# Darkkey/erlamsa

Measured on AMD Instinct MI355X. Metric: mutated_MB_per_s, higher is better.
Workload: dtype u8 (byte edits) + f64 (AS183 draws)

## Files before the change

### erlamsa_amd/csrc/eh_fuse_red.h

```cpp
#pragma once

namespace eh {

constexpr uint32_t FR_NONE = 0xFFFFFFFFu;
constexpr uint32_t FR_MAX_PERIOD = 1u << 16;
constexpr int FR_LEVELS = 4;

EH_DEV uint64_t fr_ld8(cbptr S, uint32_t q, uint32_t len) {
  uint64_t by = 0;
  if (q + 8 <= len) by = ldg8(S + q);
  else { for (uint32_t k = 0; k < 8; k++) if (q + k < len) by |= (uint64_t)S[q + k] << (8 * k); }
  return by;
}
EH_DEV uint32_t fr_peek_rounds(const Rng& r) {
  const uint32_t l = (uint32_t)EH_LANE;
  double x = rng_peek(r, l + 1u) * 8.0;
  unsigned long long z = __ballot((uint32_t)x == 0u);
  return z ? (uint32_t)__builtin_ctzll(z) : 64u;
}
__device__ __noinline__ uint32_t fr_run_fwd(cbptr S, uint32_t i0, uint32_t p, uint32_t n) {
  const uint32_t l = (uint32_t)EH_LANE;
  const uint32_t lim = n - p;
  for (uint32_t base = i0;; base += 1024) {
    const uint32_t q = base + 16u * l;
    uint32_t mp = FR_NONE;
    if (q + 16 <= lim) {
      uint4 a, b;
      a = ldg16(S + q); b = ldg16(S + q + p);
      const uint32_t x[4] = {a.x ^ b.x, a.y ^ b.y, a.z ^ b.z, a.w ^ b.w};
#pragma unroll
      for (int k = 3; k >= 0; k--) if (x[k]) mp = q + 4u * (uint32_t)k + ((uint32_t)__builtin_ctz(x[k]) >> 3);
    } else {
      for (uint32_t k = 0; k < 16; k++) { if (q + k >= lim || S[q + k] != S[q + k + p]) { mp = q + k; break; } }
    }
    unsigned long long hit = __ballot(mp != FR_NONE);
    if (hit) return (uint32_t)__builtin_amdgcn_readlane((int)mp, (int)__builtin_ctzll(hit));
  }
}
__device__ __noinline__ uint32_t fr_run_bwd(cbptr S, uint32_t i0, uint32_t p) {
  const uint32_t l = (uint32_t)EH_LANE;
  for (uint32_t hi = i0;; hi -= 1024) {
    uint32_t mp = FR_NONE;
    const uint32_t top = 16u * l < hi ? hi - 16u * l : 0u, bot = 16u * (l + 1u) < hi ? hi - 16u * (l + 1u) : 0u;
    if (top - bot == 16u) {
      uint4 a, b;
      a = ldg16(S + bot); b = ldg16(S + bot + p);
      const uint32_t x[4] = {a.x ^ b.x, a.y ^ b.y, a.z ^ b.z, a.w ^ b.w};
#pragma unroll
      for (int k = 0; k < 4; k++) if (x[k]) mp = bot + 4u * (uint32_t)k + ((31u - (uint32_t)__builtin_clz(x[k])) >> 3);
    } else {
      for (uint32_t k = bot; k < top; k++) if (S[k] != S[k + p]) mp = k;
    }
    unsigned long long hit = __ballot(mp != FR_NONE);
    if (hit) return (uint32_t)__builtin_amdgcn_readlane((int)mp, (int)__builtin_ctzll(hit)) + 1u;
    if (hi <= 1024) return 0;
  }
}
__device__ __noinline__ uint32_t fr_find8(cbptr S, uint32_t from, uint32_t lim, uint32_t n, uint64_t key) {
  const uint32_t l = (uint32_t)EH_LANE;
  if (n < 8) return FR_NONE;
  if (lim > n - 7) lim = n - 7;
  for (uint32_t base = from; base < lim; base += 1024) {
    const uint32_t q = base + 16u * l;
    uint64_t w0 = 0, w1 = 0, w2 = 0;
    if (q + 24 <= n) { w0 = ldg8(S + q); w1 = ldg8(S + q + 8); w2 = ldg8(S + q + 16); }
    else if (q < lim) { w0 = fr_ld8(S, q, n); w1 = fr_ld8(S, q + 8, n); w2 = fr_ld8(S, q + 16, n); }
    uint32_t first = 16;
#pragma unroll
    for (int k = 15; k >= 0; k--) {
      const uint64_t lo = k < 8 ? w0 : w1, hi = k < 8 ? w1 : w2;
      const int sh = 8 * (k & 7);
      const uint64_t win = sh ? (lo >> sh) | (hi << (64 - sh)) : lo;
      if (win == key && q + (uint32_t)k < lim) first = (uint32_t)k;
    }
    unsigned long long hit = __ballot(first < 16);
    if (hit) { int src = (int)__builtin_ctzll(hit); return base + 16u * (uint32_t)src + (uint32_t)__builtin_amdgcn_readlane((int)first, src); }
  }
  return FR_NONE;
}
__device__ __noinline__ bool fr_find_cut(cbptr S, uint32_t n, uint32_t R, uint32_t* cu, uint32_t* cD, uint32_t* cP = nullptr) {
  uint32_t bestD = 0, bestU = 0, blo = 0, bhi = 0, bestP = 0;
  if (n < 4096) return false;
  bool any = false;
  for (uint32_t ai = 0; ai < 7; ai++) {
    const uint32_t a = ai == 0 ? 4u : ai == 1 ? 2u : ai == 2 ? 6u : ai == 3 ? 1u : ai == 4 ? 3u : ai == 5 ? 5u : 7u;
    if (ai == 3 && !any) break;
    const uint32_t x = (uint32_t)(((uint64_t)n * a) >> 3);
    if (x + 8 > n) continue;
    if (bestD && x >= blo && x < bhi) continue;
    const uint64_t key = fr_ld8(S, x, n);
    uint32_t y = x + 1;
    for (int tries = 0; tries < 4; tries++) {
      const uint32_t far = x + 1u + FR_MAX_PERIOD < n ? x + 1u + FR_MAX_PERIOD : n;
      y = fr_find8(S, y, far, n, key);
      if (y == FR_NONE) break;
      any = true;
      const uint32_t p = y - x;
      const uint32_t hi = fr_run_fwd(S, x, p, n), lo = fr_run_bwd(S, x, p);
      const uint32_t u = lo + p, b = hi + p;
      if (b > u + R && b - u - R >= p) {
        const uint32_t D = (b - R - u) / p * p;
        if (D > bestD) { bestD = D; bestU = u; blo = lo; bhi = b; bestP = p; }
      }
      if (bestD >= n / 2) break;
      y++;
    }
    if (bestD >= n / 2) break;
  }
  if (bestD < 2048 || bestD < n / 8) return false;
  *cu = bestU; *cD = bestD;
  if (cP) *cP = bestP;
  return true;
}
__device__ __noinline__ cbptr fr_reduce(Ctx&, cbptr S, uint32_t* n, uint32_t R) {
  EH_CTX;
  uint32_t u = 0, D = 0, len = *n;
  if (!fr_find_cut(S, len, R, &u, &D)) return S;
  bptr C = ws_alloc(c, (uint64_t)len - D + 16);
  if (!C) return nullptr;
  wave_copy(C, S, u);
  wave_copy(C + u, S + u + D, len - u - D);
  len -= D;
  wave_sync();
  for (int lv = 1; lv < FR_LEVELS; lv++) {
    if (!fr_find_cut(C, len, R, &u, &D)) break;
    wave_sync();
    wave_move_down(C + u, C + u + D, len - u - D);
    len -= D;
    wave_sync();
// ... 60 lines not shown
```

### erlamsa_amd/csrc/eh_sgml.h

```cpp
#pragma once
#include "eh_doc.h"

namespace eh {

enum { E_LT = 1, E_GT, E_WS, E_EQ, E_SL, E_SQ, E_DQ, E_DASH, E_QM, E_BANG, E_SLGT, E_QGT, E_CMTEND, E_SPACE };
constexpr uint32_t ES_WS = (1u << E_WS) | (1u << E_SPACE);
constexpr uint32_t ES_EV = ES_WS | (1u << E_GT) | (1u << E_EQ);
constexpr uint32_t ES_STOP = ES_EV | (1u << E_SLGT);
constexpr uint32_t ES_DASH = (1u << E_DASH) | (1u << E_CMTEND);
EH_DEV uint32_t sg_class(uint32_t b) {
  const uint64_t t0 = ((uint64_t)E_WS << 36) | ((uint64_t)E_WS << 40) | ((uint64_t)E_WS << 52);
  const uint64_t t2 = ((uint64_t)E_SPACE << 0) | ((uint64_t)E_BANG << 4) | ((uint64_t)E_DQ << 8) | ((uint64_t)E_SQ << 28) | ((uint64_t)E_DASH << 52) | ((uint64_t)E_SL << 60);
  const uint64_t t3 = ((uint64_t)E_LT << 48) | ((uint64_t)E_EQ << 52) | ((uint64_t)E_GT << 56) | ((uint64_t)E_QM << 60);
  uint64_t t = b < 16 ? t0 : (b < 32 ? 0ull : (b < 48 ? t2 : t3));
  return b < 64 ? (uint32_t)((t >> (4 * (b & 15))) & 15) : 0u;
}

__constant__ uint8_t c_sglit[24] = {'<', '>', ' ', '=', '\'', '"', '<', '/', ' ', '/', '>', '<', '?', '?', '>', '<', '!', '<', '!', '-', '-', '-', '-', '>'};
enum { SL_LT = 0, SL_GT = 1, SL_SP = 2, SL_EQ = 3, SL_SQ = 4, SL_DQ = 5, SL_LTSL = 6, SL_SPSLGT = 8, SL_LTQ = 11, SL_QGT = 13, SL_LTBANG = 15, SL_CMT = 17, SL_CMTEND = 21 };
EH_DEV cbptr sglit(int k) { return (cbptr)&c_sglit[k]; }

enum { TK_OPEN = 1, TK_CLOSE = 2, TK_SC = 3, TK_TEXT = 4, TK_BANG = 5, TK_COMMENT = 6, TK_QUE = 7, TK_KIND = 0xFF, TF_EMPTY = 0x100, TF_PAIRED = 0x200 };
struct SgTok { uint32_t kind, p0, np, na, nb, par0, npar; int32_t match; };
struct SgParam { uint32_t na, nb, va, vb, delim, pad; };
// ... 224 lines not shown
        R.va = pos + 1; R.vb = EV(jq) >> 4; R.delim = cv == E_SQ ? 1u : 2u;
        pos = R.vb + 1; ei = jq + 1;
      } else {
        const uint32_t ju = find_stop(ei);
        if (ju >= nev || bail) break;
        R.va = pos; R.vb = EV(ju) >> 4; pos = R.vb; ei = ju;
      }
      skipws();
    }
    if (bail) break;
    R.term = 0; R.npos = pos; R.nei = ei; R.nws = ws_sp ? 1u : 0u;
  } while (false);
  R.reach = reach;
  return R;
}

__device__ __noinline__ int sgml_tokenize(Ctx&, cbptr H, uint32_t L, SgDoc* out) {
  EH_CTX;
  const int l = EH_LANE;
#ifdef EH_PROF
  const uint64_t ph1_t0 = __builtin_readcyclecounter();
#endif
  wptr ev = (wptr)ws_alloc(c, ((uint64_t)L + 80) * 4);
  if (!ev) return -3;
  uint32_t nev = 0, nlt = 0, nstop = 0;
  for (uint32_t tb = 0; tb < L; tb += 1024) {
    uint32_t i0 = tb + 16u * (uint32_t)l;
    uint8_t b[18];
    if (i0 + 18 <= L) { uint4 v = ldg16(H + i0); __builtin_memcpy(b, &v, 16); b[16] = H[i0 + 16]; b[17] = H[i0 + 17]; }
    else { for (uint32_t k = 0; k < 18; k++) b[k] = i0 + k < L ? H[i0 + k] : 0; }
    uint32_t cls[16]; uint32_t cnt = 0, lts = 0, stops = 0;
#pragma unroll
    for (uint32_t k = 0; k < 16; k++) {
      uint32_t x = b[k];
      uint32_t cl = i0 + k < L ? sg_class(x) : 0u;
      if (cl == E_SL && b[k + 1] == '>') cl = E_SLGT;
      if (cl == E_QM && b[k + 1] == '>') cl = E_QGT;
      if (cl == E_DASH && b[k + 1] == '-' && b[k + 2] == '>') cl = E_CMTEND;
      cls[k] = cl; cnt += cl ? 1u : 0u; lts += cl == E_LT ? 1u : 0u; stops += (cl == E_WS || cl == E_SPACE || cl == E_GT || cl == E_EQ || cl == E_SL || cl == E_SLGT) ? 1u : 0u;
    }
    uint32_t inc = wave_incl_scan(cnt);
    uint32_t o = nev + inc - cnt;
#pragma unroll
    for (uint32_t k = 0; k < 16; k++) if (cls[k]) ev[o++] = ((i0 + k) << 4) | cls[k];
    nev += (uint32_t)__builtin_amdgcn_readlane((int)inc, 63);
    nlt += lts; nstop += stops;
  }
  nlt = wave_sum(nlt); nstop = wave_sum(nstop);
#ifdef EH_PROF
  uint64_t sub_t0 = __builtin_readcyclecounter();
#define SG_SUB0() do { sub_t0 = __builtin_readcyclecounter(); } while (0)
#define SG_SUB(k) do { uint64_t n_ = __builtin_readcyclecounter(); if (l == 0) { atomicAdd(&c.p->prof[2 * (k)], (unsigned long long)(n_ - sub_t0)); atomicAdd(&c.p->prof[2 * (k) + 1], 1ull); } sub_t0 = n_; } while (0)
#define SG_CNT(k, v) do { if (l == 0) { atomicAdd(&c.p->prof[2 * (k)], (unsigned long long)(v)); atomicAdd(&c.p->prof[2 * (k) + 1], 1ull); } } while (0)
  if (l == 0) { atomicAdd(&c.p->prof[2 * 117], (unsigned long long)(sub_t0 - ph1_t0)); atomicAdd(&c.p->prof[2 * 117 + 1], 1ull); atomicAdd(&c.p->prof[2 * 119], (unsigned long long)nev); atomicAdd(&c.p->prof[2 * 119 + 1], (unsigned long long)L); }
  uint64_t tz_t0 = __builtin_readcyclecounter();
#define SG_TZ(k) do { uint64_t n_ = __builtin_readcyclecounter(); if (l == 0) { atomicAdd(&c.p->prof[2 * (k)], (unsigned long long)(n_ - tz_t0)); atomicAdd(&c.p->prof[2 * (k) + 1], 1ull); } tz_t0 = n_; } while (0)
#else
#define SG_TZ(k) do {} while (0)
#define SG_SUB0() do {} while (0)
#define SG_SUB(k) do {} while (0)
#define SG_CNT(k, v) do {} while (0)
#endif
  if (nlt == 0) return -1;
  uint32_t cap_tok = 2 * nlt + 8, cap_par = nstop + 8;
  uint64_t cap_pc = 4ull * cap_tok + (uint64_t)SG_PARPCS * cap_par + nlt + 32;
  EH_G SgTok* tok = (EH_G SgTok*)ws_alloc(c, (uint64_t)cap_tok * sizeof(SgTok));
  EH_G SgParam* par = (EH_G SgParam*)ws_alloc(c, (uint64_t)cap_par * sizeof(SgParam));
  EH_G Piece* pc = (EH_G Piece*)ws_alloc(c, cap_pc * sizeof(Piece));
  if (!tok || !par || !pc) return -3;
  wave_sync();
  uint32_t ntok = 0, npar = 0, npc = 0;

  constexpr uint32_t SG_EVC = 4096, SG_EVBACK = 512;
  uint32_t cbase = 0xFFFFFFFFu;
  uint32_t bev = 0, bbase = 0xFFFFFFFFu;
  uint32_t reach_ev = 0;
  auto need = [&](uint32_t i) {
    if (bbase != 0xFFFFFFFFu && i >= bbase && i < bbase + 64) return;
    bbase = i & ~63u;
    if (bbase + 64 > reach_ev) reach_ev = bbase + 64;
    if (cbase == 0xFFFFFFFFu || bbase < cbase || bbase + 64 > cbase + SG_EVC) {
      cbase = bbase > SG_EVBACK ? bbase - SG_EVBACK : 0u;
      lanes_sync();
      for (uint32_t k0 = 0; k0 < SG_EVC; k0 += 256) {
        uint32_t v[4];
#pragma unroll
        for (int u = 0; u < 4; u++) { uint32_t j = cbase + k0 + 64u * (uint32_t)u + (uint32_t)l; v[u] = j < nev ? ev[j] : 0u; }
#pragma unroll
        for (int u = 0; u < 4; u++) g_fuse_lds[k0 + 64u * (uint32_t)u + (uint32_t)l] = v[u];
      }
      lanes_sync();
    }
    bev = g_fuse_lds[bbase - cbase + (uint32_t)l];
  };
  auto find = [&](uint32_t from, uint32_t set) -> uint32_t {
    while (from < nev) {
      need(from);
      unsigned long long m = __ballot(((set >> (bev & 15u)) & 1u) != 0 && bbase + (uint32_t)l >= from && bbase + (uint32_t)l < nev);
      if (m) return bbase + (uint32_t)__builtin_ctzll(m);
      from = bbase + 64;
    }
    return nev;
  };
  auto evget = [&](uint32_t i) -> uint32_t { need(i); return (uint32_t)__builtin_amdgcn_readlane((int)bev, (int)(i - bbase)); };
  uint32_t ff_gt = nev, ff_qgt = nev, ff_cmt = nev, ff_sq = nev, ff_dq = nev;
  auto find1 = [&](uint32_t from, uint32_t cls, uint32_t& ff) -> uint32_t {
    if (from >= ff) return nev;
// ... 1014 lines not shown
```

### erlamsa_amd/csrc/eh_text.h

```cpp
#pragma once
#include "eh_device.h"

namespace eh {

template <class Pred>
EH_DEV uint32_t tile_mask(cbptr p, uint32_t n, uint32_t tile_base, Pred pred) {
  uint32_t i0 = tile_base + 16u * (uint32_t)EH_LANE;
  if (i0 >= n) return 0;
  uint32_t cnt = n - i0 < 16 ? n - i0 : 16;
  uint8_t b[16];
  if (cnt == 16) { uint4 v = ldg16(p + i0); __builtin_memcpy(b, &v, 16); }
  else { for (uint32_t k = 0; k < 16; k++) b[k] = k < cnt ? p[i0 + k] : 0; }
  uint32_t prev = i0 > 0 ? p[i0 - 1] : 256u;
  uint32_t m = 0;
#pragma unroll
  for (uint32_t k = 0; k < 16; k++) {
    if (k < cnt && pred((uint32_t)b[k], prev)) m |= 1u << k;
    prev = b[k];
  }
  return m;
}
EH_DEV uint32_t wave_incl_scan(uint32_t v) {
  const int l = EH_LANE;
#pragma unroll
  for (int d = 1; d < 64; d <<= 1) { uint32_t t = __shfl_up(v, d); if (l >= d) v += t; }
  return v;
}
EH_DEV uint32_t wave_sum(uint32_t v) {
#pragma unroll
  for (int d = 32; d > 0; d >>= 1) v += __shfl_xor(v, d);
  return uni(v);
}
template <class Pred>
EH_DEV uint32_t wave_count(cbptr p, uint32_t n, Pred pred) {
  uint32_t c = 0;
  for (uint32_t tb = 0; tb < n; tb += 1024) c += __popc(tile_mask(p, n, tb, pred));
  return wave_sum(c);
}
template <class Pred>
EH_DEV uint32_t wave_find_kth(cbptr p, uint32_t n, uint32_t k, Pred pred) {
  uint32_t before = 0;
  for (uint32_t tb = 0; tb < n; tb += 1024) {
    uint32_t m = tile_mask(p, n, tb, pred);
    uint32_t inc = wave_incl_scan(__popc(m));
    uint32_t tile_total = uni((uint32_t)__shfl(inc, 63));
    if (k < before + tile_total) {
      uint32_t kk = k - before;
      bool mine = inc > kk && inc - __popc(m) <= kk;
      unsigned long long who = __ballot(mine);
      int src = (int)__builtin_ctzll(who);
      uint32_t pos = 0;
      if (mine) {
        uint32_t r = kk - (inc - __popc(m));
        uint32_t mm = m;
        for (uint32_t t = 0; t < r; t++) mm &= mm - 1;
        pos = tb + 16u * (uint32_t)EH_LANE + (uint32_t)__builtin_ctz(mm);
      }
      return uni((uint32_t)__shfl(pos, src));
    }
    before += tile_total;
  }
  return n;
}
template <class Pred>
EH_DEV void wave_collect(cbptr p, uint32_t n, uint32_t r0, uint32_t r1, wptr out, Pred pred) {
  uint32_t before = 0;
  for (uint32_t tb = 0; tb < n && before < r1; tb += 1024) {
    uint32_t m = tile_mask(p, n, tb, pred);
    uint32_t inc = wave_incl_scan(__popc(m));
    uint32_t rank = before + inc - __popc(m);
    uint32_t mm = m;
    while (mm) {
      uint32_t bit = (uint32_t)__builtin_ctz(mm); mm &= mm - 1;
      if (rank >= r0 && rank < r1) out[rank - r0] = tb + 16u * (uint32_t)EH_LANE + bit;
      rank++;
    }
    before += uni((uint32_t)__shfl(inc, 63));
  }
  wave_sync();
}

EH_DEV bool binarish(cbptr p, uint32_t n) {
  const int l = EH_LANE;
  uint32_t mine = (uint32_t)l < n && l < 11 ? p[l] : 0;
  uint32_t b[11];
#pragma unroll
  for (int k = 0; k < 11; k++) b[k] = (uint32_t)__builtin_amdgcn_readlane((int)mine, k);
#pragma unroll
  for (uint32_t pos = 0; pos <= 8; pos++) {
    uint32_t rem = n > pos ? n - pos : 0;
    if (rem >= 3 && b[pos] == 0xEF && b[pos + 1] == 0xBB && b[pos + 2] == 0xBF) return false;
    if (rem >= 2 && b[pos] == 0xFE && b[pos + 1] == 0x0F) return false;
    if (pos == 8) return false;
    if (rem == 0) return false;
    if (b[pos] == 0) return true;
    if (b[pos] & 128) return true;
  }
  return false;
}

struct Pieces {
  uint64_t p[6]; uint32_t n[6]; uint32_t rep[6]; int k;
};
EH_DEV void pc_init(Pieces& q) { q.k = 0; }
EH_DEV void pc_add(Pieces& q, cbptr p, uint32_t n, uint32_t rep = 1) { q.p[q.k] = (uint64_t)p; q.n[q.k] = n; q.rep[q.k] = rep; q.k++; }
EH_DEV bool pc_emit(Ctx& c, const Pieces& q) {
  uint64_t total = 0;
#pragma unroll
  for (int i = 0; i < 6; i++) if (i < q.k) total += (uint64_t)q.n[i] * q.rep[i];
  if (total > 0xFFFFFFF0ull) { EH_SET_OVERFLOW(c, 701); return false; }
  bptr dst = ws_alloc(c, total);
  if (!dst) return false;
  uint64_t pos = 0;
#pragma unroll
  for (int i = 0; i < 6; i++) if (i < q.k) {
    if (q.rep[i] == 1) wave_copy(dst + pos, (cbptr)q.p[i], q.n[i]);
    else wave_fill_periodic(dst + pos, (cbptr)q.p[i], q.n[i], (uint64_t)q.n[i] * q.rep[i]);
    pos += (uint64_t)q.n[i] * q.rep[i];
  }
  wave_sync();
  c.r_kind = R_NEW; c.r_ptr = dst; c.r_len = (uint32_t)total;
  return true;
}

struct IsNl { EH_DEV bool operator()(uint32_t b, uint32_t) const { return b == 10; } };

struct LineIdx {
  cbptr p; uint32_t L, nnl, N;
};
EH_DEV void li_init(LineIdx& li, cbptr p, uint32_t L) {
// ... 497 lines not shown
```

### erlamsa_amd/csrc/eh_tree.h

```cpp
#pragma once
#include "eh_lex.h"

namespace eh {

struct TNode { uint32_t open, close, pend, pad; };

EH_DEV uint32_t usual_delim_close(uint32_t c) {
  switch (c) { case 40: return 41; case 91: return 93; case 60: return 62; case 123: return 125; case 34: return 34; case 39: return 39; }
  return 0;
}
struct DelimCls {
  EH_DEV uint32_t operator()(uint32_t b) const {
    switch (b) { case 40: return 1; case 41: return 2; case 91: return 3; case 93: return 4; case 60: return 5; case 62: return 6;
                 case 123: return 7; case 125: return 8; case 34: return 9; case 39: return 10; }
    return 0;
  }
};
EH_DEV uint32_t delim_close_code(uint32_t code) { return code == 9 ? 9u : (code == 10 ? 10u : code + 1); }
EH_DEV bool delim_is_opener(uint32_t code) { return code == 1 || code == 3 || code == 5 || code == 7 || code == 9 || code == 10; }
EH_DEV bool delim_bit(uint32_t b, uint32_t w1, uint32_t w23) { uint32_t m = b < 32 ? 0u : (b < 64 ? w1 : (b < 128 ? w23 : 0u)); return (m >> (b & 31u)) & 1u; }
struct IsOpener { EH_DEV bool operator()(uint32_t b, uint32_t) const { return delim_bit(b, (1u << 2) | (1u << 7) | (1u << 8) | (1u << 28), 1u << 27); } };

#ifndef EH_TREE_S
#define EH_TREE_S 32
#endif
constexpr uint32_t TL_S = EH_TREE_S;
constexpr uint32_t TL_SP = TL_S + 4;
constexpr uint32_t TL_COD = 0;
constexpr uint32_t TL_LNK = TL_COD + 16 * TL_SP;
constexpr uint32_t TL_STK = TL_LNK + 16 * TL_SP;
constexpr uint32_t TL_TOP = TL_STK + 32 * TL_S;
constexpr uint32_t TL_ESC = TL_TOP + 64 * TL_S;
constexpr uint32_t TL_TAIL = 4 * TL_S;
constexpr uint32_t TL_SEQ_MIN = 1024, TL_SEQ_MAX = 65536;
static_assert(TL_S >= 8 && TL_S <= 32 && TL_S % 4 == 0, "tree_parse: per-run event masks are 32 bits wide");
static_assert(TL_ESC + 16 * TL_SP <= EH_FUSE_LDS_WORDS, "g_fuse_lds too small for the lane batches of tree_parse");
EH_DEV uint8_t* tl_bytes() { return reinterpret_cast<uint8_t*>(g_fuse_lds); }
EH_DEV uint16_t* tl_stack() { return reinterpret_cast<uint16_t*>(g_fuse_lds + TL_STK); }
#ifdef EH_PROF
#define TR_PH(k) do { uint64_t now_ = __builtin_readcyclecounter(); if (EH_LANE == 0) { atomicAdd(&c.p->prof[2 * (70 + (k))], (unsigned long long)(now_ - tph)); atomicAdd(&c.p->prof[2 * (70 + (k)) + 1], 1ull); } tph = now_; } while (0)
#define TR_ST(k, v) do { if (EH_LANE == 0) { atomicAdd(&c.p->prof[2 * (70 + (k))], (unsigned long long)(v)); atomicAdd(&c.p->prof[2 * (70 + (k)) + 1], 1ull); } } while (0)
#else
#define TR_PH(k) do { } while (0)
#define TR_ST(k, v) do { } while (0)
#endif
#ifdef HIPEMU
extern "C" { inline unsigned long long eh_emu_tree_lanes[5] = {0, 0, 0, 0, 0}; }
#define TL_COUNT(i, v) do { if (EH_LANE == 0) eh_emu_tree_lanes[i] += (v); } while (0)
#else
#define TL_COUNT(i, v) do { } while (0)
#endif
struct IsDelim { EH_DEV bool operator()(uint32_t b, uint32_t) const { return delim_bit(b, (1u << 2) | (1u << 7) | (1u << 8) | (1u << 9) | (1u << 28) | (1u << 30), (1u << 27) | (1u << 29)); } };
EH_DEV void delim_tile_masks(cbptr p, uint32_t n, uint32_t tile_base, uint32_t& md, uint32_t& mo, uint32_t& mq) {
  md = 0; mo = 0; mq = 0;
  uint32_t i0 = tile_base + 16u * (uint32_t)EH_LANE;
  if (i0 >= n) return;
  uint32_t cnt = n - i0 < 16 ? n - i0 : 16;
  uint8_t b[16];
  if (cnt == 16) { uint4 v = ldg16(p + i0); __builtin_memcpy(b, &v, 16); }
  else { for (uint32_t k = 0; k < 16; k++) b[k] = k < cnt ? p[i0 + k] : 0; }
#pragma unroll
  for (uint32_t k = 0; k < 16; k++) {
    if (IsDelim()((uint32_t)b[k], 0)) md |= 1u << k;
    if (IsOpener()((uint32_t)b[k], 0)) mo |= 1u << k;
#ifdef EH_PROF
    if (b[k] == 34 || b[k] == 39) mq |= 1u << k;
#endif
  }
}
__device__ __noinline__ int tree_parse(Ctx&, cbptr H, uint32_t L, EH_G TNode** out) {
  EH_CTX;
  const int l = EH_LANE;
#ifdef EH_PROF
  uint64_t tph = __builtin_readcyclecounter();
#endif
  uint32_t nev = 0, nopen = 0, nquote = 0;
  for (uint32_t tb = 0; tb < L; tb += 1024) { uint32_t md, mo, mq; delim_tile_masks(H, L, tb, md, mo, mq); nev += __popc(md); nopen += __popc(mo); nquote += __popc(mq); }
  nev = wave_sum(nev); nopen = wave_sum(nopen);
#ifdef EH_PROF
  nquote = wave_sum(nquote);
#endif
  EH_G TNode* tab = (EH_G TNode*)ws_alloc(c, (uint64_t)(nopen + 1) * sizeof(TNode));
  wptr spill = (wptr)ws_alloc(c, (uint64_t)(nopen + 64) * 4);
  wptr evp = (wptr)ws_alloc(c, (uint64_t)(nev + 64) * 4);
  if (!tab || !spill || !evp) return -1;
  if (nopen >= (1u << 24)) { EH_SET_OVERFLOW(c, 801); return -1; }
  TR_PH(10);
  wave_collect(H, L, 0, nev, evp, IsDelim());
  TR_PH(11); TR_ST(15, nev);
  for (uint32_t i = (uint32_t)l; i < nopen + 1; i += 64) tab[i].close = 0xFFFFFFFFu;
  wave_sync();
  uint32_t stk = 0;
  uint32_t sp = 0, sbase = 0;
  uint32_t top = 0;
  uint32_t orank = 0;
  auto rs_refill = [&]() {
    uint32_t up = (uint32_t)__shfl_up((int)stk, 32);
    sbase -= 32;
    stk = l < 32 ? spill[sbase + l] : up;
  };
  auto rs_spill = [&]() {
    if (l < 32) spill[sbase + l] = stk;
    stk = (uint32_t)__shfl_down((int)stk, 32);
    sbase += 32;
  };
  auto rs_pop = [&]() {
    sp--;
    if (sp > 0) {
      if (sp == sbase) rs_refill();
      top = (uint32_t)__builtin_amdgcn_readlane((int)stk, (int)(sp - 1 - sbase));
    }
  };
  auto rs_push = [&](uint32_t ent) {
    if (sp - sbase == 64) rs_spill();
    if ((uint32_t)l == sp - sbase) stk = ent;
    top = ent; sp++;
  };
  const bool lanes_on = !(c.p->flags & EH_FLAG_TREE_NO_LANES) && nev >= 8 * TL_S;
  uint32_t seq_left = 0, seq_len = TL_SEQ_MIN;
  uint32_t nlane = 0;
  if (lanes_on) { TL_COUNT(3, 1); TL_COUNT(4, nev); }
  uint32_t eb = 0;
  while (eb < nev) {
    eb = uni(eb); sp = uni(sp); sbase = uni(sbase); top = uni(top); orank = uni(orank); seq_left = uni(seq_left); seq_len = uni(seq_len);
    if (!lanes_on || seq_left > 0 || nev - eb < TL_TAIL) {
      uint32_t mycode = eb + (uint32_t)l < nev ? DelimCls()((uint32_t)H[evp[eb + l]]) : 0;
      mycode |= delim_is_opener(mycode) ? (0x100u | (delim_close_code(mycode) << 16)) : 0u;
      uint32_t cnt = nev - eb < 64 ? nev - eb : 64;
      const unsigned long long opm = __ballot((mycode & 0x100u) != 0);
      uint32_t npush = 0, nclose = 0;
// ... 150 lines not shown
        const uint32_t rb = ob + (uint32_t)__popc(okm & ((1u << sj) - 1));
        for (uint32_t e2 = 0; e2 < rem; e2++) {
          const uint32_t code = (uint32_t)__builtin_amdgcn_readlane((int)mc, (int)e2);
          if (sp > 0 && (code & 255u) == (top & 255u)) {
            if ((uint32_t)l == nclose) { cs = top >> 8; ce = ev0 + sj + e2; }
            nclose++;
            rs_pop();
            if (nclose == 64) w_flush();
          } else if (code & 0x100u) {
            const uint32_t parent = sp > 0 ? top >> 8 : 0xFFFFFFFFu;
            const uint32_t slot = rb + (uint32_t)__popcll(opm & ((1ull << e2) - 1));
            if ((uint32_t)l == npush) { ps = slot; pe = ev0 + sj + e2; pp = parent; }
            npush++;
            rs_push((slot << 8) | (code >> 16));
            if (npush == 64) w_flush();
          }
        }
        nseq += rem;
      }
      if (l == k) topout = sp > 0 ? top >> 8 : 0xFFFFFFFFu;
    }
    w_flush();
    lanes_sync();
    {
      const unsigned long long below = items & ((1ull << l) - 1);
      const uint32_t t = (uint32_t)__shfl((int)topout, below ? 63 - (int)__builtin_clzll(below) : 0);
      if (!((items >> l) & 1ull)) topin = below ? t : top0;
    }
    {
      const uint32_t lb = 4 * TL_LNK + (uint32_t)l * TL_SP, ev0 = eb + (uint32_t)l * TL_S;
      uint32_t m = cm;
      while (m) {
        const uint32_t j = (uint32_t)__builtin_ctz(m); m &= m - 1;
        const uint32_t jo = tl_bytes()[lb + j], lp = tl_bytes()[lb + jo];
        const uint32_t slot = obase + (uint32_t)__popc(om & ((1u << jo) - 1));
        uint32_t par;
        if (lp != 255u) par = obase + (uint32_t)__popc(om & ((1u << lp) - 1));
        else { const uint32_t e = (uint32_t)__popc(em & ((1u << jo) - 1)); par = e ? g_fuse_lds[TL_TOP + (uint32_t)l * TL_S + e - 1] : topin; }
        tab[slot].open = ev0 + jo; tab[slot].close = ev0 + j; tab[slot].pend = par;
      }
    }
    orank += (uint32_t)__builtin_amdgcn_readlane((int)oinc, 63);
    eb += committed;
    nlane += committed - nseq; TL_COUNT(0, committed - nseq); TL_COUNT(1, 1);
    if (2 * nseq > committed) { TL_COUNT(2, 1); seq_left = seq_len; if (seq_len < TL_SEQ_MAX) seq_len *= 2; }
    else if (seq_len > TL_SEQ_MIN) seq_len /= 2;
  }
  wave_sync();
  TR_PH(12);
#ifdef EH_PROF
  if (l == 0) { atomicAdd(&c.p->prof[2 * 86], (unsigned long long)nlane); atomicAdd(&c.p->prof[2 * 86 + 1], (unsigned long long)nquote); }
#endif
  (void)nlane; (void)nquote;
  for (uint32_t i = (uint32_t)l; i < nopen; i += 64) {
    if (tab[i].close == 0xFFFFFFFFu) continue;
    uint32_t par = tab[i].pend, pe = L;
    if (par != 0xFFFFFFFFu) { uint32_t pc = tab[par].close; if (pc != 0xFFFFFFFFu) pe = evp[pc] + 1; }
    tab[i].pad = pe;
  }
  wave_sync();
  TR_PH(13);
  uint32_t n = 0;
  for (uint32_t base = 0; base < nopen; base += 64) {
    uint32_t i = base + (uint32_t)l;
    TNode t{0, 0xFFFFFFFFu, 0, 0};
    if (i < nopen) t = tab[i];
    bool ok = i < nopen && t.close != 0xFFFFFFFFu;
    unsigned long long m = __ballot(ok);
    uint32_t before = (uint32_t)__popcll(m & ((1ull << l) - 1));
    wave_sync();
    if (ok) { t.open = evp[t.open]; t.close = evp[t.close]; t.pend = t.pad; tab[n + before] = t; }
    n += (uint32_t)__popcll(m);
    wave_sync();
  }
  TR_PH(14);
  *out = tab;
  return (int)n;
}

EH_DEV bool node_eq(cbptr H, TNode a, TNode b) {
  uint32_t la = a.close - a.open + 1, lb = b.close - b.open + 1;
  if (la != lb) return false;
  if (a.open == b.open) return true;
  return wave_equal(H + a.open, H + b.open, la);
}
EH_DEV TNode node_load(const EH_G TNode* t, uint32_t i) { TNode x = t[i]; x.open = uni(x.open); x.close = uni(x.close); x.pend = uni(x.pend); return x; }

EH_DEV unsigned long long nodes_equal_mask(cbptr H, uint32_t my_open, bool cand, TNode sub) {
  uint32_t n = sub.close - sub.open + 1;
  if (n > 256) {
    unsigned long long cm = __ballot(cand), res = 0;
    while (cm) {
      int j = (int)__builtin_ctzll(cm); cm &= cm - 1;
      uint32_t o = (uint32_t)__builtin_amdgcn_readlane((int)my_open, j);
      if (o == sub.open || wave_equal(H + o, H + sub.open, n)) res |= 1ull << j;
    }
    return res;
  }
  bool ne = !cand;
  bool self = cand && my_open == sub.open;
  uint32_t k = 0;
  for (; k + 8 <= n; k += 8) {
    uint64_t a = 0, b;
    b = ldg8(H + sub.open + k);
    if (!ne && !self) a = ldg8(H + my_open + k);
    ne = ne || (!self && a != b);
    if (__ballot(!ne && !self) == 0) break;
  }
  if (k + 8 <= n) return __ballot(!ne);
  for (; k < n; k++) { uint32_t b = H[sub.open + k]; if (!ne && !self && H[my_open + k] != b) ne = true; }
  return __ballot(!ne);
}
template <class F>
EH_DEV void tree_matches(cbptr H, const EH_G TNode* nodes, uint32_t lo, uint32_t hi, uint32_t level_end, TNode sub, wptr anc, F f) {
  (void)anc;
  const int l = EH_LANE;
  (void)l;
  uint32_t skip_until = 0;
  uint32_t slen = sub.close - sub.open;
  for (uint32_t base = lo; base < hi; base += 64) {
    uint32_t i = base + (uint32_t)l;
    TNode q{0, 0, 0, 0};
    if (i < hi) q = nodes[i];
    bool cand = i < hi && q.close - q.open == slen && q.open >= skip_until;
    if (__ballot(cand) == 0) continue;
// ... 279 lines not shown
```

Before: 96240.

## Batch global loads across multiple tiles in scan, run and compaction loops

Several wave-level byte-scanning loops (run extension forward/backward, 8-byte key search, delimiter/predicate tile masks) now issue loads for several 1 KiB tiles up front and then consume them in order, so more memory requests are in flight per wave. Tree node finalisation and compaction loops are likewise unrolled four-wide so the dependent gathers through tab and evp overlap. The predicate scan also takes the previous byte from a lane shuffle instead of a separate global load. In exchange, register pressure rises and some bytes past an early exit are loaded for nothing. A profiling counter index is also changed under EH_PROF.

```diff
diff --git a/erlamsa_amd/csrc/eh_fuse_red.h b/erlamsa_amd/csrc/eh_fuse_red.h
--- a/erlamsa_amd/csrc/eh_fuse_red.h
+++ b/erlamsa_amd/csrc/eh_fuse_red.h
@@ -5,6 +5,7 @@
 constexpr uint32_t FR_NONE = 0xFFFFFFFFu;
 constexpr uint32_t FR_MAX_PERIOD = 1u << 16;
 constexpr int FR_LEVELS = 4;
+constexpr int FR_RUN_TILES = 2;
 
 EH_DEV uint64_t fr_ld8(cbptr S, uint32_t q, uint32_t len) {
   uint64_t by = 0;
@@ -21,60 +22,97 @@
 __device__ __noinline__ uint32_t fr_run_fwd(cbptr S, uint32_t i0, uint32_t p, uint32_t n) {
   const uint32_t l = (uint32_t)EH_LANE;
   const uint32_t lim = n - p;
-  for (uint32_t base = i0;; base += 1024) {
-    const uint32_t q = base + 16u * l;
-    uint32_t mp = FR_NONE;
-    if (q + 16 <= lim) {
-      uint4 a, b;
-      a = ldg16(S + q); b = ldg16(S + q + p);
-      const uint32_t x[4] = {a.x ^ b.x, a.y ^ b.y, a.z ^ b.z, a.w ^ b.w};
-#pragma unroll
-      for (int k = 3; k >= 0; k--) if (x[k]) mp = q + 4u * (uint32_t)k + ((uint32_t)__builtin_ctz(x[k]) >> 3);
-    } else {
-      for (uint32_t k = 0; k < 16; k++) { if (q + k >= lim || S[q + k] != S[q + k + p]) { mp = q + k; break; } }
-    }
-    unsigned long long hit = __ballot(mp != FR_NONE);
-    if (hit) return (uint32_t)__builtin_amdgcn_readlane((int)mp, (int)__builtin_ctzll(hit));
+  for (uint32_t base = i0;; base += 1024u * FR_RUN_TILES) {
+    uint4 a[FR_RUN_TILES], b[FR_RUN_TILES];
+#pragma unroll
+    for (int u = 0; u < FR_RUN_TILES; u++) {
+      const uint32_t q = base + 1024u * (uint32_t)u + 16u * l;
+      a[u].x = a[u].y = a[u].z = a[u].w = 0; b[u] = a[u];
+      if (q + 16 <= lim) { a[u] = ldg16(S + q); b[u] = ldg16(S + q + p); }
+    }
+#pragma unroll
+    for (int u = 0; u < FR_RUN_TILES; u++) {
+      const uint32_t q = base + 1024u * (uint32_t)u + 16u * l;
+      uint32_t mp = FR_NONE;
+      if (q + 16 <= lim) {
+        const uint32_t x[4] = {a[u].x ^ b[u].x, a[u].y ^ b[u].y, a[u].z ^ b[u].z, a[u].w ^ b[u].w};
+#pragma unroll
+        for (int k = 3; k >= 0; k--) if (x[k]) mp = q + 4u * (uint32_t)k + ((uint32_t)__builtin_ctz(x[k]) >> 3);
+      } else {
+        for (uint32_t k = 0; k < 16; k++) { if (q + k >= lim || S[q + k] != S[q + k + p]) { mp = q + k; break; } }
+      }
+      unsigned long long hit = __ballot(mp != FR_NONE);
+      if (hit) return (uint32_t)__builtin_amdgcn_readlane((int)mp, (int)__builtin_ctzll(hit));
+    }
   }
 }
 __device__ __noinline__ uint32_t fr_run_bwd(cbptr S, uint32_t i0, uint32_t p) {
   const uint32_t l = (uint32_t)EH_LANE;
-  for (uint32_t hi = i0;; hi -= 1024) {
-    uint32_t mp = FR_NONE;
-    const uint32_t top = 16u * l < hi ? hi - 16u * l : 0u, bot = 16u * (l + 1u) < hi ? hi - 16u * (l + 1u) : 0u;
-    if (top - bot == 16u) {
-      uint4 a, b;
-      a = ldg16(S + bot); b = ldg16(S + bot + p);
-      const uint32_t x[4] = {a.x ^ b.x, a.y ^ b.y, a.z ^ b.z, a.w ^ b.w};
-#pragma unroll
-      for (int k = 0; k < 4; k++) if (x[k]) mp = bot + 4u * (uint32_t)k + ((31u - (uint32_t)__builtin_clz(x[k])) >> 3);
-    } else {
-      for (uint32_t k = bot; k < top; k++) if (S[k] != S[k + p]) mp = k;
-    }
-    unsigned long long hit = __ballot(mp != FR_NONE);
-    if (hit) return (uint32_t)__builtin_amdgcn_readlane((int)mp, (int)__builtin_ctzll(hit)) + 1u;
-    if (hi <= 1024) return 0;
+  for (uint32_t ghi = i0;; ghi -= 1024u * FR_RUN_TILES) {
+    uint4 a[FR_RUN_TILES], b[FR_RUN_TILES];
+#pragma unroll
+    for (int u = 0; u < FR_RUN_TILES; u++) {
+      const uint32_t hi = ghi > 1024u * (uint32_t)u ? ghi - 1024u * (uint32_t)u : 0u;
+      const uint32_t top = 16u * l < hi ? hi - 16u * l : 0u, bot = 16u * (l + 1u) < hi ? hi - 16u * (l + 1u) : 0u;
+      a[u].x = a[u].y = a[u].z = a[u].w = 0; b[u] = a[u];
+      if (top - bot == 16u) { a[u] = ldg16(S + bot); b[u] = ldg16(S + bot + p); }
+    }
+#pragma unroll
+    for (int u = 0; u < FR_RUN_TILES; u++) {
+      const uint32_t hi = ghi > 1024u * (uint32_t)u ? ghi - 1024u * (uint32_t)u : 0u;
+      const uint32_t top = 16u * l < hi ? hi - 16u * l : 0u, bot = 16u * (l + 1u) < hi ? hi - 16u * (l + 1u) : 0u;
+      uint32_t mp = FR_NONE;
+      if (top - bot == 16u) {
+        const uint32_t x[4] = {a[u].x ^ b[u].x, a[u].y ^ b[u].y, a[u].z ^ b[u].z, a[u].w ^ b[u].w};
+#pragma unroll
+        for (int k = 0; k < 4; k++) if (x[k]) mp = bot + 4u * (uint32_t)k + ((31u - (uint32_t)__builtin_clz(x[k])) >> 3);
+      } else {
+        for (uint32_t k = bot; k < top; k++) if (S[k] != S[k + p]) mp = k;
+      }
+      unsigned long long hit = __ballot(mp != FR_NONE);
+      if (hit) return (uint32_t)__builtin_amdgcn_readlane((int)mp, (int)__builtin_ctzll(hit)) + 1u;
+      if (hi <= 1024) return 0;
+    }
   }
 }
 __device__ __noinline__ uint32_t fr_find8(cbptr S, uint32_t from, uint32_t lim, uint32_t n, uint64_t key) {
   const uint32_t l = (uint32_t)EH_LANE;
   if (n < 8) return FR_NONE;
   if (lim > n - 7) lim = n - 7;
-  for (uint32_t base = from; base < lim; base += 1024) {
-    const uint32_t q = base + 16u * l;
-    uint64_t w0 = 0, w1 = 0, w2 = 0;
-    if (q + 24 <= n) { w0 = ldg8(S + q); w1 = ldg8(S + q + 8); w2 = ldg8(S + q + 16); }
-    else if (q < lim) { w0 = fr_ld8(S, q, n); w1 = fr_ld8(S, q + 8, n); w2 = fr_ld8(S, q + 16, n); }
-    uint32_t first = 16;
-#pragma unroll
-    for (int k = 15; k >= 0; k--) {
-      const uint64_t lo = k < 8 ? w0 : w1, hi = k < 8 ? w1 : w2;
-      const int sh = 8 * (k & 7);
-      const uint64_t win = sh ? (lo >> sh) | (hi << (64 - sh)) : lo;
-      if (win == key && q + (uint32_t)k < lim) first = (uint32_t)k;
-    }
-    unsigned long long hit = __ballot(first < 16);
-    if (hit) { int src = (int)__builtin_ctzll(hit); return base + 16u * (uint32_t)src + (uint32_t)__builtin_amdgcn_readlane((int)first, src); }
+  for (uint32_t gb = from; gb < lim; gb += 4096) {
+    uint64_t w0[4], w1[4], w2[4];
+    uint32_t tu = 4;
+#pragma unroll
+    for (int u = 0; u < 4; u++) {
+      const uint32_t q = gb + 1024u * (uint32_t)u + 16u * l;
+      w0[u] = w1[u] = w2[u] = 0;
+      if (q < lim) {
+        if (q + 24 <= n) { w0[u] = ldg8(S + q); w1[u] = ldg8(S + q + 8); w2[u] = ldg8(S + q + 16); }
+        else tu = (uint32_t)u;
+      }
+    }
+    if (tu < 4) {
+      const uint32_t q = gb + 1024u * tu + 16u * l;
+      const uint64_t t0 = fr_ld8(S, q, n), t1 = fr_ld8(S, q + 8, n), t2 = fr_ld8(S, q + 16, n);
+#pragma unroll
+      for (uint32_t u = 0; u < 4; u++) if (tu == u) { w0[u] = t0; w1[u] = t1; w2[u] = t2; }
+    }
+#pragma unroll 1
+    for (uint32_t base = gb; base < gb + 4096u && base < lim; base += 1024) {
+      const uint32_t q = base + 16u * l;
+      uint32_t first = 16;
+#pragma unroll
+      for (int k = 15; k >= 0; k--) {
+        const uint64_t lo = k < 8 ? w0[0] : w1[0], hi = k < 8 ? w1[0] : w2[0];
+        const int sh = 8 * (k & 7);
+        const uint64_t win = sh ? (lo >> sh) | (hi << (64 - sh)) : lo;
+        if (win == key && q + (uint32_t)k < lim) first = (uint32_t)k;
+      }
+      unsigned long long hit = __ballot(first < 16);
+      if (hit) { int src = (int)__builtin_ctzll(hit); return base + 16u * (uint32_t)src + (uint32_t)__builtin_amdgcn_readlane((int)first, src); }
+#pragma unroll
+      for (int u = 0; u < 3; u++) { w0[u] = w0[u + 1]; w1[u] = w1[u + 1]; w2[u] = w2[u + 1]; }
+    }
   }
   return FR_NONE;
 }
diff --git a/erlamsa_amd/csrc/eh_sgml.h b/erlamsa_amd/csrc/eh_sgml.h
--- a/erlamsa_amd/csrc/eh_sgml.h
+++ b/erlamsa_amd/csrc/eh_sgml.h
@@ -300,7 +300,7 @@
 #define SG_SUB0() do { sub_t0 = __builtin_readcyclecounter(); } while (0)
 #define SG_SUB(k) do { uint64_t n_ = __builtin_readcyclecounter(); if (l == 0) { atomicAdd(&c.p->prof[2 * (k)], (unsigned long long)(n_ - sub_t0)); atomicAdd(&c.p->prof[2 * (k) + 1], 1ull); } sub_t0 = n_; } while (0)
 #define SG_CNT(k, v) do { if (l == 0) { atomicAdd(&c.p->prof[2 * (k)], (unsigned long long)(v)); atomicAdd(&c.p->prof[2 * (k) + 1], 1ull); } } while (0)
-  if (l == 0) { atomicAdd(&c.p->prof[2 * 117], (unsigned long long)(sub_t0 - ph1_t0)); atomicAdd(&c.p->prof[2 * 117 + 1], 1ull); atomicAdd(&c.p->prof[2 * 119], (unsigned long long)nev); atomicAdd(&c.p->prof[2 * 119 + 1], (unsigned long long)L); }
+  if (l == 0) { atomicAdd(&c.p->prof[2 * 96], (unsigned long long)(sub_t0 - ph1_t0)); atomicAdd(&c.p->prof[2 * 96 + 1], 1ull); atomicAdd(&c.p->prof[2 * 119], (unsigned long long)nev); atomicAdd(&c.p->prof[2 * 119 + 1], (unsigned long long)L); }
   uint64_t tz_t0 = __builtin_readcyclecounter();
 #define SG_TZ(k) do { uint64_t n_ = __builtin_readcyclecounter(); if (l == 0) { atomicAdd(&c.p->prof[2 * (k)], (unsigned long long)(n_ - tz_t0)); atomicAdd(&c.p->prof[2 * (k) + 1], 1ull); } tz_t0 = n_; } while (0)
 #else
diff --git a/erlamsa_amd/csrc/eh_text.h b/erlamsa_amd/csrc/eh_text.h
--- a/erlamsa_amd/csrc/eh_text.h
+++ b/erlamsa_amd/csrc/eh_text.h
@@ -3,15 +3,48 @@
 
 namespace eh {
 
+constexpr uint32_t TG_BYTES = 4096;
+struct TileGroup { uint4 v[4]; uint32_t pb; };
+
+EH_DEV uint32_t tile_cnt(uint32_t n, uint32_t tile_base) {
+  const uint32_t i0 = tile_base + 16u * (uint32_t)EH_LANE;
+  return i0 >= n ? 0u : (n - i0 < 16 ? n - i0 : 16u);
+}
+EH_DEV void tg_load(TileGroup& g, cbptr p, uint32_t n, uint32_t base) {
+  const uint32_t l = (uint32_t)EH_LANE;
+  g.pb = 256u;
+  if (l == 0 && base > 0) g.pb = p[base - 1];
+#pragma unroll
+  for (int u = 0; u < 4; u++) {
+    const uint32_t i0 = base + 1024u * (uint32_t)u + 16u * l;
+    g.v[u].x = g.v[u].y = g.v[u].z = g.v[u].w = 0;
+    if (i0 < n && n - i0 >= 16) g.v[u] = ldg16(p + i0);
+  }
+  const uint32_t t0 = n & ~15u, tn = n & 15u;
+  if (tn && t0 >= base && t0 - base < TG_BYTES && (((t0 - base) >> 4) & 63u) == l) {
+    uint8_t b[16];
+    for (uint32_t k = 0; k < 16; k++) b[k] = k < tn ? p[t0 + k] : 0;
+    uint4 t; __builtin_memcpy(&t, b, 16);
+    const uint32_t tu = (t0 - base) >> 10;
+#pragma unroll
+    for (uint32_t u = 0; u < 4; u++) if (tu == u) g.v[u] = t;
+  }
+}
+EH_DEV uint4 tg_pop(TileGroup& g) {
+  const uint4 v = g.v[0];
+  g.pb = (uint32_t)__builtin_amdgcn_readlane((int)v.w, 63) >> 24;
+  g.v[0] = g.v[1]; g.v[1] = g.v[2]; g.v[2] = g.v[3];
+  return v;
+}
 template <class Pred>
-EH_DEV uint32_t tile_mask(cbptr p, uint32_t n, uint32_t tile_base, Pred pred) {
-  uint32_t i0 = tile_base + 16u * (uint32_t)EH_LANE;
-  if (i0 >= n) return 0;
-  uint32_t cnt = n - i0 < 16 ? n - i0 : 16;
+EH_DEV uint32_t tg_mask(TileGroup& g, uint32_t n, uint32_t tile_base, Pred pred) {
+  const uint32_t cnt = tile_cnt(n, tile_base);
+  const uint32_t pb = g.pb;
+  const uint4 v = tg_pop(g);
   uint8_t b[16];
-  if (cnt == 16) { uint4 v = ldg16(p + i0); __builtin_memcpy(b, &v, 16); }
-  else { for (uint32_t k = 0; k < 16; k++) b[k] = k < cnt ? p[i0 + k] : 0; }
-  uint32_t prev = i0 > 0 ? p[i0 - 1] : 256u;
+  __builtin_memcpy(b, &v, 16);
+  uint32_t prev = (uint32_t)__shfl_up((int)(v.w >> 24), 1);
+  if (EH_LANE == 0) prev = pb;
   uint32_t m = 0;
 #pragma unroll
   for (uint32_t k = 0; k < 16; k++) {
@@ -34,48 +67,60 @@
 template <class Pred>
 EH_DEV uint32_t wave_count(cbptr p, uint32_t n, Pred pred) {
   uint32_t c = 0;
-  for (uint32_t tb = 0; tb < n; tb += 1024) c += __popc(tile_mask(p, n, tb, pred));
+  for (uint32_t base = 0; base < n; base += TG_BYTES) {
+    TileGroup g; tg_load(g, p, n, base);
+#pragma unroll 1
+    for (uint32_t tb = base; tb < base + TG_BYTES && tb < n; tb += 1024) c += __popc(tg_mask(g, n, tb, pred));
+  }
   return wave_sum(c);
 }
 template <class Pred>
 EH_DEV uint32_t wave_find_kth(cbptr p, uint32_t n, uint32_t k, Pred pred) {
   uint32_t before = 0;
-  for (uint32_t tb = 0; tb < n; tb += 1024) {
-    uint32_t m = tile_mask(p, n, tb, pred);
-    uint32_t inc = wave_incl_scan(__popc(m));
-    uint32_t tile_total = uni((uint32_t)__shfl(inc, 63));
-    if (k < before + tile_total) {
-      uint32_t kk = k - before;
-      bool mine = inc > kk && inc - __popc(m) <= kk;
-      unsigned long long who = __ballot(mine);
-      int src = (int)__builtin_ctzll(who);
-      uint32_t pos = 0;
-      if (mine) {
-        uint32_t r = kk - (inc - __popc(m));
-        uint32_t mm = m;
-        for (uint32_t t = 0; t < r; t++) mm &= mm - 1;
-        pos = tb + 16u * (uint32_t)EH_LANE + (uint32_t)__builtin_ctz(mm);
-      }
-      return uni((uint32_t)__shfl(pos, src));
-    }
-    before += tile_total;
+  for (uint32_t base = 0; base < n; base += TG_BYTES) {
+    TileGroup g; tg_load(g, p, n, base);
+#pragma unroll 1
+    for (uint32_t tb = base; tb < base + TG_BYTES && tb < n; tb += 1024) {
+      uint32_t m = tg_mask(g, n, tb, pred);
+      uint32_t inc = wave_incl_scan(__popc(m));
+      uint32_t tile_total = uni((uint32_t)__shfl(inc, 63));
+      if (k < before + tile_total) {
+        uint32_t kk = k - before;
+        bool mine = inc > kk && inc - __popc(m) <= kk;
+        unsigned long long who = __ballot(mine);
+        int src = (int)__builtin_ctzll(who);
+        uint32_t pos = 0;
+        if (mine) {
+          uint32_t r = kk - (inc - __popc(m));
+          uint32_t mm = m;
+          for (uint32_t t = 0; t < r; t++) mm &= mm - 1;
+          pos = tb + 16u * (uint32_t)EH_LANE + (uint32_t)__builtin_ctz(mm);
+        }
+        return uni((uint32_t)__shfl(pos, src));
+      }
+      before += tile_total;
+    }
   }
   return n;
 }
 template <class Pred>
 EH_DEV void wave_collect(cbptr p, uint32_t n, uint32_t r0, uint32_t r1, wptr out, Pred pred) {
   uint32_t before = 0;
-  for (uint32_t tb = 0; tb < n && before < r1; tb += 1024) {
-    uint32_t m = tile_mask(p, n, tb, pred);
-    uint32_t inc = wave_incl_scan(__popc(m));
-    uint32_t rank = before + inc - __popc(m);
-    uint32_t mm = m;
-    while (mm) {
-      uint32_t bit = (uint32_t)__builtin_ctz(mm); mm &= mm - 1;
-      if (rank >= r0 && rank < r1) out[rank - r0] = tb + 16u * (uint32_t)EH_LANE + bit;
-      rank++;
-    }
-    before += uni((uint32_t)__shfl(inc, 63));
+  for (uint32_t base = 0; base < n && before < r1; base += TG_BYTES) {
+    TileGroup g; tg_load(g, p, n, base);
+#pragma unroll 1
+    for (uint32_t tb = base; tb < base + TG_BYTES && tb < n && before < r1; tb += 1024) {
+      uint32_t m = tg_mask(g, n, tb, pred);
+      uint32_t inc = wave_incl_scan(__popc(m));
+      uint32_t rank = before + inc - __popc(m);
+      uint32_t mm = m;
+      while (mm) {
+        uint32_t bit = (uint32_t)__builtin_ctz(mm); mm &= mm - 1;
+        if (rank >= r0 && rank < r1) out[rank - r0] = tb + 16u * (uint32_t)EH_LANE + bit;
+        rank++;
+      }
+      before += uni((uint32_t)__shfl(inc, 63));
+    }
   }
   wave_sync();
 }
diff --git a/erlamsa_amd/csrc/eh_tree.h b/erlamsa_amd/csrc/eh_tree.h
--- a/erlamsa_amd/csrc/eh_tree.h
+++ b/erlamsa_amd/csrc/eh_tree.h
@@ -51,14 +51,11 @@
 #define TL_COUNT(i, v) do { } while (0)
 #endif
 struct IsDelim { EH_DEV bool operator()(uint32_t b, uint32_t) const { return delim_bit(b, (1u << 2) | (1u << 7) | (1u << 8) | (1u << 9) | (1u << 28) | (1u << 30), (1u << 27) | (1u << 29)); } };
-EH_DEV void delim_tile_masks(cbptr p, uint32_t n, uint32_t tile_base, uint32_t& md, uint32_t& mo, uint32_t& mq) {
+EH_DEV void delim_tile_masks(TileGroup& g, uint32_t& md, uint32_t& mo, uint32_t& mq) {
   md = 0; mo = 0; mq = 0;
-  uint32_t i0 = tile_base + 16u * (uint32_t)EH_LANE;
-  if (i0 >= n) return;
-  uint32_t cnt = n - i0 < 16 ? n - i0 : 16;
+  const uint4 v = tg_pop(g);
   uint8_t b[16];
-  if (cnt == 16) { uint4 v = ldg16(p + i0); __builtin_memcpy(b, &v, 16); }
-  else { for (uint32_t k = 0; k < 16; k++) b[k] = k < cnt ? p[i0 + k] : 0; }
+  __builtin_memcpy(b, &v, 16);
 #pragma unroll
   for (uint32_t k = 0; k < 16; k++) {
     if (IsDelim()((uint32_t)b[k], 0)) md |= 1u << k;
@@ -75,7 +72,11 @@
   uint64_t tph = __builtin_readcyclecounter();
 #endif
   uint32_t nev = 0, nopen = 0, nquote = 0;
-  for (uint32_t tb = 0; tb < L; tb += 1024) { uint32_t md, mo, mq; delim_tile_masks(H, L, tb, md, mo, mq); nev += __popc(md); nopen += __popc(mo); nquote += __popc(mq); }
+  for (uint32_t base = 0; base < L; base += TG_BYTES) {
+    TileGroup g; tg_load(g, H, L, base);
+#pragma unroll 1
+    for (uint32_t tb = base; tb < base + TG_BYTES && tb < L; tb += 1024) { uint32_t md, mo, mq; delim_tile_masks(g, md, mo, mq); nev += __popc(md); nopen += __popc(mo); nquote += __popc(mq); }
+  }
   nev = wave_sum(nev); nopen = wave_sum(nopen);
 #ifdef EH_PROF
   nquote = wave_sum(nquote);
@@ -332,25 +333,46 @@
   if (l == 0) { atomicAdd(&c.p->prof[2 * 86], (unsigned long long)nlane); atomicAdd(&c.p->prof[2 * 86 + 1], (unsigned long long)nquote); }
 #endif
   (void)nlane; (void)nquote;
-  for (uint32_t i = (uint32_t)l; i < nopen; i += 64) {
-    if (tab[i].close == 0xFFFFFFFFu) continue;
-    uint32_t par = tab[i].pend, pe = L;
-    if (par != 0xFFFFFFFFu) { uint32_t pc = tab[par].close; if (pc != 0xFFFFFFFFu) pe = evp[pc] + 1; }
-    tab[i].pad = pe;
+  for (uint32_t base = 0; base < nopen; base += 256) {
+    uint32_t cl[4], par[4], pc[4], pe[4];
+#pragma unroll
+    for (int u = 0; u < 4; u++) {
+      const uint32_t i = base + 64u * (uint32_t)u + (uint32_t)l;
+      cl[u] = par[u] = 0xFFFFFFFFu;
+      if (i < nopen) { cl[u] = tab[i].close; par[u] = tab[i].pend; }
+    }
+#pragma unroll
+    for (int u = 0; u < 4; u++) { pc[u] = 0xFFFFFFFFu; if (cl[u] != 0xFFFFFFFFu && par[u] != 0xFFFFFFFFu) pc[u] = tab[par[u]].close; }
+#pragma unroll
+    for (int u = 0; u < 4; u++) { pe[u] = L; if (pc[u] != 0xFFFFFFFFu) pe[u] = evp[pc[u]] + 1; }
+#pragma unroll
+    for (int u = 0; u < 4; u++) {
+      const uint32_t i = base + 64u * (uint32_t)u + (uint32_t)l;
+      if (cl[u] != 0xFFFFFFFFu) tab[i].pad = pe[u];
+    }
   }
   wave_sync();
   TR_PH(13);
   uint32_t n = 0;
-  for (uint32_t base = 0; base < nopen; base += 64) {
-    uint32_t i = base + (uint32_t)l;
-    TNode t{0, 0xFFFFFFFFu, 0, 0};
-    if (i < nopen) t = tab[i];
-    bool ok = i < nopen && t.close != 0xFFFFFFFFu;
-    unsigned long long m = __ballot(ok);
-    uint32_t before = (uint32_t)__popcll(m & ((1ull << l) - 1));
+  for (uint32_t base = 0; base < nopen; base += 256) {
+    TNode t[4]; bool ok[4]; uint32_t po[4], pcl[4];
+#pragma unroll
+    for (int u = 0; u < 4; u++) {
+      const uint32_t i = base + 64u * (uint32_t)u + (uint32_t)l;
+      t[u] = TNode{0, 0xFFFFFFFFu, 0, 0};
+      if (i < nopen) t[u] = tab[i];
+      ok[u] = i < nopen && t[u].close != 0xFFFFFFFFu;
+    }
+#pragma unroll
+    for (int u = 0; u < 4; u++) { po[u] = pcl[u] = 0; if (ok[u]) { po[u] = evp[t[u].open]; pcl[u] = evp[t[u].close]; } }
     wave_sync();
-    if (ok) { t.open = evp[t.open]; t.close = evp[t.close]; t.pend = t.pad; tab[n + before] = t; }
-    n += (uint32_t)__popcll(m);
+#pragma unroll
+    for (int u = 0; u < 4; u++) {
+      unsigned long long m = __ballot(ok[u]);
+      uint32_t before = (uint32_t)__popcll(m & ((1ull << l) - 1));
+      if (ok[u]) { t[u].open = po[u]; t[u].close = pcl[u]; t[u].pend = t[u].pad; tab[n + before] = t[u]; }
+      n += (uint32_t)__popcll(m);
+    }
     wave_sync();
   }
   TR_PH(14);
```

After: 96610, median of 3. No clear change (+0.4%).
